# stevenmiller888/mlx-audio

Measured on AMD Instinct MI355X. Metric: audio-sec/sec (xRT), Kokoro-82M batch=32 fixed 128-phoneme utterances per GPU, higher is better.
Workload: dtype bf16; 1 GPU; Kokoro-82M bf16, batch=32/GPU fixed 128-phoneme utterances (T=130, F=650, 390000 samples = 16.25 s each), utterance-sharded over 1 GPU(s); global_batch=32, parallelism=utterance-shard x1, 2 batches in flight per GPU

## Files before the change

include/kokoro_hip.h:

```cpp
#ifndef KOKORO_HIP_H
#define KOKORO_HIP_H

#include <stddef.h>
#include <stdint.h>

#ifdef __cplusplus
extern "C" {
#endif

#define KK_ABI_VERSION 2
#define KK_ABI_MINOR 3

enum { KK_DTYPE_F32 = 0, KK_DTYPE_BF16 = 1, KK_DTYPE_I32 = 2, KK_DTYPE_F16 = 3 };
enum { KK_NOISE_ZERO = 0, KK_NOISE_INJECTED = 1, KK_NOISE_PHILOX = 2 };

typedef struct kk_model kk_model;
typedef struct kk_context kk_context;

typedef struct kk_config {
  int32_t n_token, hidden_dim, style_dim, n_layer, max_dur, text_encoder_kernel_size;
  int32_t plbert_hidden, plbert_heads, plbert_intermediate, plbert_max_pos, plbert_layers, plbert_embedding;
  int32_t decoder_hidden;
  int32_t upsample_initial_channel;
  int32_t n_upsamples;
// ... 23 lines not shown
int kk_forward_text(kk_context* cx, void* stream, int B, int Tmax, const int32_t* ids, const int32_t* lens, const float* ref_s,
                    const float* speed, void* workspace, size_t workspace_bytes, int32_t* pred_dur_out);

int kk_forward_audio(kk_context* cx, void* stream, int B, int Tmax, const int32_t* lens, const float* ref_s, const int32_t* dur, int Fmax,
                     int noise_mode, const float* sine_noise, uint64_t seed, void* workspace, size_t workspace_bytes, float* wav_out,
                     int32_t* nframes_out);

int kk_forward(kk_context* cx, void* stream, int B, int Tmax, const int32_t* ids, const int32_t* lens, const float* ref_s, const float* speed,
               const int32_t* forced_dur, int Fmax, int noise_mode, const float* sine_noise, uint64_t seed, void* workspace,
               size_t workspace_bytes, float* wav_out, int32_t* pred_dur_out, int32_t* nframes_out);

int kk_set_graph_mode(kk_context* cx, int on);

int kk_set_quantization(kk_model* m, int group_size, int bits);
int kk_quantized_layers(const kk_model* m);

const char* kk_last_error(void);
int kk_abi_version(void);
int kk_abi_minor(void);


int kk_op_conv1d(void* stream, int B, const void* x, int ldx, int Lin_rows, const int32_t* lin, const float* w_packed, int ldw,
                 const float* bias, int Cin, int Cout, int Kw, int transposed, int stride, int pad, int dil, int in_shift, float in_slope,
                 int act, float act_slope, const void* res, int ldr, float scale, int accumulate, void* out, int ldo, int Lout_rows,
                 const int32_t* lout, int in_dtype, int out_dtype);
int kk_op_conv1d_bf16(void* stream, int B, const void* x, int ldx, int Lin_rows, const int32_t* lin, const void* w_bf16, int CinP, int CoutP,
                      const float* bias, int Cout, int Kw, int transposed, int stride, int pad, int dil, int in_shift, float in_slope,
                      int act, float act_slope, const void* res, int ldr, float scale, int accumulate, void* out, int ldo, int Lout_rows,
                      const int32_t* lout, int out_dtype);
int kk_op_conv1d_bf16_fused(void* stream, int B, const void* x, int ldx, int L_rows, const int32_t* len, const void* w_bf16, int CinP,
                            int CoutP, const float* bias, int Cin, int Cout, int Kw, int pad, int dil, const float* nrm_a,
                            const float* nrm_b, int nrm_stride, int nrm_act, float nrm_slope, const float* nrm_alpha, const void* res,
                            int ldr, float scale, void* out, int ldo, float* stat_part, int* stat_ntiles_out);
int kk_op_adain(void* stream, int B, const void* x, int ldx, int L_rows, const int32_t* len, int C, const float* gamma_beta, int gbs,
                int act, float slope, const float* alpha, int pool, const float* pool_w, const float* pool_b, void* out, int ldo, int Cpad,
                int Lout_rows, float* scratch, size_t scratch_floats, int dtype, int fast);
int kk_op_layernorm(void* stream, int B, const void* x, int ldx, const void* res, int ldr, int L_rows, const int32_t* len, int C,
                    const float* w, const float* b, const float* gamma_beta, int gbs, float eps, int act, float slope, void* out, int ldo,
                    int dtype);
int kk_op_lstm(void* stream, int B, const float* xproj, const float* whT, int H, int L_rows, const int32_t* len, void* out, int ldo,
               int dtype);
int kk_op_linear_rows(void* stream, int B, const void* x_bf16, long long xbs, int ldx, int rows, const int32_t* len, const void* w_bf16, int N, int K,
                      const float* bias, int act, void* pack_scratch, void* out_bf16, long long obs, int ldo);
int kk_op_lstm_bf16(void* stream, int B, const float* xproj, const void* wh_bf16, int L_rows, const int32_t* len, void* out, int ldo,
                    int dtype);
int kk_op_attention(void* stream, int B, const void* qkv, int ld, int T_rows, const int32_t* len, int heads, void* out, int ldo, int dtype);
int kk_op_source_stft(void* stream, int B, const float* f0, int L2_rows, const int32_t* len2, const float* lin_w9, float lin_b,
                      int noise_mode, const float* noise, uint64_t seed, float* phase_scratch, float* har_source, void* har, int ldhar,
                      int dtype);
int kk_op_istft_head(void* stream, int B, const void* x, int ldx, int Tf_rows, const int32_t* len_frames, float* wav, int dtype, int fast);
int kk_op_pack_head_w(void* stream, const void* w_bf16, void* w_frag);
int kk_op_conv_post_istft(void* stream, int B, const void* x, int ldx, int Tf_rows, const int32_t* len_frames, const void* w_frag,
                          const float* bias, float in_slope, float* wav, void* cp_out, int cp_ld);

int kk_mxfp8_bytes(int rows, int K, size_t* q_bytes, size_t* s_bytes);
int kk_mxfp8_pack_weight(const float* w_host, int N, int K, int group, uint8_t* q_host, uint8_t* s_host);
int kk_op_linear_mxfp8(void* stream, const void* x_bf16, int ldx, int M, int rows_per_item, const int32_t* len, int K, const void* wq,
                       const void* ws, int N, const float* bias, int act, void* aq, void* as, void* out_bf16, int ldo);

int kk_debug_info(kk_context* cx, const char* name, int64_t* rows, int64_t* channels);
int kk_debug_fetch(kk_context* cx, void* stream, const char* name, float* dst);
int kk_debug_override(kk_context* cx, const char* name, const float* src);
void kk_debug_clear(kk_context* cx);
int kk_op_pack_w_frag(void* stream, const void* w_bf16, void* w_frag, int Kw, int CoutP, int CinP);
void kk_debug_set_op_wfrag(const void* w_frag);
void kk_debug_set_op_variant(int v);
// ... 125 lines not shown
```

mlx-audio_amd/_lib.py:

```python
from __future__ import annotations

import ctypes as C
import os

_HERE = os.path.dirname(os.path.abspath(__file__))
LIB_PATH = os.path.join(_HERE, "libkokoro_hip.so")

KK_F32, KK_BF16, KK_I32, KK_F16 = 0, 1, 2, 3
CSM_WEIGHTS = {0: "f32", 1: "bf16", 2: "q8", 3: "q4"}
CSM_WEIGHTS_MIXED, CSM_WEIGHTS_DEQUANTIZED = 0x100, 0x200
NOISE_ZERO, NOISE_INJECTED, NOISE_PHILOX = 0, 1, 2
ACT_NONE, ACT_LRELU, ACT_GELU, ACT_SNAKE = 0, 1, 2, 3


class KKConfig(C.Structure):
    _fields_ = [
        ("n_token", C.c_int32), ("hidden_dim", C.c_int32), ("style_dim", C.c_int32), ("n_layer", C.c_int32),
        ("max_dur", C.c_int32), ("text_encoder_kernel_size", C.c_int32),
        ("plbert_hidden", C.c_int32), ("plbert_heads", C.c_int32), ("plbert_intermediate", C.c_int32),
        ("plbert_max_pos", C.c_int32), ("plbert_layers", C.c_int32), ("plbert_embedding", C.c_int32),
        ("decoder_hidden", C.c_int32), ("upsample_initial_channel", C.c_int32), ("n_upsamples", C.c_int32),
        ("upsample_rates", C.c_int32 * 4), ("upsample_kernel_sizes", C.c_int32 * 4),
        ("n_resblock_kernels", C.c_int32), ("resblock_kernel_sizes", C.c_int32 * 4),
        ("resblock_dilations", (C.c_int32 * 3) * 4),
# ... 17 lines not shown


class KKCsmConfig(C.Structure):
    _fields_ = [("text_vocab_size", C.c_int32), ("audio_vocab_size", C.c_int32), ("audio_num_codebooks", C.c_int32), ("max_seq_len", C.c_int32),
                ("backbone", KKLlamaArgs), ("decoder", KKLlamaArgs)]


class KKCsmSampler(C.Structure):
    _fields_ = [("temperature", C.c_float), ("top_k", C.c_int32), ("top_p", C.c_float), ("min_p", C.c_float), ("min_tokens_to_keep", C.c_int32),
                ("seed", C.c_uint64), ("use_device_rng", C.c_int32)]


_vp, _i, _f, _sz, _u64 = C.c_void_p, C.c_int, C.c_float, C.c_size_t, C.c_uint64
SIGNATURES = {
    "kk_create": (_i, [C.POINTER(KKConfig), C.POINTER(_vp)]),
    "kk_destroy": (None, [_vp]),
    "kk_load_tensor": (_i, [_vp, C.c_char_p, _i, C.POINTER(C.c_int64), _i, _vp]),
    "kk_finalize": (_i, [_vp, _vp]),
    "kk_workspace_bytes": (_sz, [_vp, _i, _i, _i]),
    "kk_context_create": (_i, [_vp, C.POINTER(_vp)]),
    "kk_context_destroy": (None, [_vp]),
    "kk_context_model": (_vp, [_vp]),
    "kk_context_workspace_bytes": (_sz, [_vp, _i, _i, _i]),
    "kk_forward_text": (_i, [_vp, _vp, _i, _i, _vp, _vp, _vp, _vp, _vp, _sz, _vp]),
    "kk_forward_audio": (_i, [_vp, _vp, _i, _i, _vp, _vp, _vp, _i, _i, _vp, _u64, _vp, _sz, _vp, _vp]),
    "kk_forward": (_i, [_vp, _vp, _i, _i, _vp, _vp, _vp, _vp, _vp, _i, _i, _vp, _u64, _vp, _sz, _vp, _vp, _vp]),
    "kk_last_error": (C.c_char_p, []),
    "kk_abi_version": (_i, []),
    "kk_abi_minor": (_i, []),
    "kk_op_conv1d": (_i, [_vp, _i, _vp, _i, _i, _vp, _vp, _i, _vp, _i, _i, _i, _i, _i, _i, _i, _i, _f, _i, _f, _vp, _i, _f, _i, _vp, _i, _i, _vp, _i, _i]),
    "kk_op_conv1d_bf16": (_i, [_vp, _i, _vp, _i, _i, _vp, _vp, _i, _i, _vp, _i, _i, _i, _i, _i, _i, _i, _f, _i, _f, _vp, _i, _f, _i, _vp, _i, _i, _vp, _i]),
    "kk_op_conv1d_bf16_fused": (_i, [_vp, _i, _vp, _i, _i, _vp, _vp, _i, _i, _vp, _i, _i, _i, _i, _i, _vp, _vp, _i, _i, _f, _vp, _vp, _i, _f,
                                     _vp, _i, _vp, C.POINTER(C.c_int)]),
    "kk_op_adain": (_i, [_vp, _i, _vp, _i, _i, _vp, _i, _vp, _i, _i, _f, _vp, _i, _vp, _vp, _vp, _i, _i, _i, _vp, _sz, _i, _i]),
    "kk_op_layernorm": (_i, [_vp, _i, _vp, _i, _vp, _i, _i, _vp, _i, _vp, _vp, _vp, _i, _f, _i, _f, _vp, _i, _i]),
    "kk_op_lstm": (_i, [_vp, _i, _vp, _vp, _i, _i, _vp, _vp, _i, _i]),
    "kk_op_lstm_bf16": (_i, [_vp, _i, _vp, _vp, _i, _vp, _vp, _i, _i]),
    "kk_op_linear_rows": (_i, [_vp, _i, _vp, C.c_longlong, _i, _i, _vp, _vp, _i, _i, _vp, _i, _vp, _vp, C.c_longlong, _i]),
    "kk_op_attention": (_i, [_vp, _i, _vp, _i, _i, _vp, _i, _vp, _i, _i]),
    "kk_op_source_stft": (_i, [_vp, _i, _vp, _i, _vp, _vp, _f, _i, _vp, _u64, _vp, _vp, _vp, _i, _i]),
    "kk_op_istft_head": (_i, [_vp, _i, _vp, _i, _i, _vp, _vp, _i, _i]),
    "kk_op_pack_head_w": (_i, [_vp, _vp, _vp]),
    "kk_op_conv_post_istft": (_i, [_vp, _i, _vp, _i, _i, _vp, _vp, _vp, _f, _vp, _vp, _i]),
    "kk_debug_info": (_i, [_vp, C.c_char_p, C.POINTER(C.c_int64), C.POINTER(C.c_int64)]),
    "kk_debug_fetch": (_i, [_vp, _vp, C.c_char_p, _vp]),
    "kk_debug_override": (_i, [_vp, C.c_char_p, _vp]),
    "kk_debug_clear": (None, [_vp]),
    "kk_debug_force_generic": (None, [_vp, _i]),
    "kk_op_pack_w_frag": (_i, [_vp, _vp, _vp, _i, _i, _i]),
    "kk_csm_create": (_i, [C.POINTER(KKCsmConfig), C.POINTER(_vp)]),
    "kk_csm_destroy": (None, [_vp]),
    "kk_csm_load_tensor": (_i, [_vp, C.c_char_p, C.POINTER(C.c_int64), _i, _vp]),
    "kk_csm_set_weight_dtype": (_i, [_vp, _i]),
    "kk_csm_load_quantized": (_i, [_vp, C.c_char_p, C.POINTER(C.c_int64), _vp, _vp, _vp, _i, _i]),
    "kk_csm_weight_format": (_i, [_vp]),
    "kk_csm_weight_fallback_reason": (C.c_char_p, [_vp]),
    "kk_csm_weight_bytes": (_i, [_vp, C.POINTER(_sz), C.POINTER(_sz)]),
    "kk_csm_finalize": (_i, [_vp, _vp]),
    "kk_csm_share": (_i, [_vp, C.POINTER(_vp)]),
    "kk_csm_setup_caches": (_i, [_vp, _i]),
    "kk_csm_reset_caches": (_i, [_vp]),
    "kk_csm_position": (_i, [_vp]),
    "kk_csm_set_padding": (_i, [_vp, _i, _vp]),
    "kk_csm_workspace_bytes": (_sz, [_vp, _i, _i]),
    "kk_csm_generate_frame": (_i, [_vp, _vp, _i, _i, _vp, _vp, _f, _i, _vp, _vp, _sz, _vp]),
    "kk_csm_generate_frame_ex": (_i, [_vp, _vp, _i, _i, _vp, _vp, C.POINTER(KKCsmSampler), _vp, _vp, _vp, _sz, _vp]),
# ... 96 lines not shown
```

mlx-audio_amd/csrc/kk_conv_mfma5.hip:

```cpp
#include <stdlib.h>

#include "kk_common.h"
#include "kk_kernels.h"
#include "kk_conv_mfma_shared.h"

#ifdef KK_MFMA_TRACE
__device__ unsigned long long kk_mfma5_trace_acc[256][8];
#define TR5_NOW() (__builtin_readcyclecounter())
#define TR5_ADD(slot, v) \
  do { if ((threadIdx.x & 255) == 0) atomicAdd(&kk_mfma5_trace_acc[blockIdx.x & 255][slot], (unsigned long long)(v)); } while (0)
extern "C" int kk_debug_mfma5_trace(unsigned long long* out8, int reset) {
  static unsigned long long h[256][8];
  if (out8) {
    if (hipMemcpyFromSymbol(h, HIP_SYMBOL(kk_mfma5_trace_acc), sizeof(h)) != hipSuccess) return -1;
    for (int k = 0; k < 8; ++k) out8[k] = 0;
    for (int r = 0; r < 256; ++r)
      for (int k = 0; k < 8; ++k) out8[k] += h[r][k];
  }
  if (reset) {
    for (int r = 0; r < 256; ++r)
      for (int k = 0; k < 8; ++k) h[r][k] = 0;
    if (hipMemcpyToSymbol(HIP_SYMBOL(kk_mfma5_trace_acc), h, sizeof(h)) != hipSuccess) return -1;
  }
  return 0;
// ... 261 lines not shown
      unsigned wq[4] = {xreg[i].x & msk & cm[0], xreg[i].y & msk & cm[1], xreg[i].z & msk & cm[2], xreg[i].w & msk & cm[3]};
      if (NRM != 0) {
      } else if (a.in_act == KK_ACT_ELU) {
#pragma unroll
        for (int k = 0; k < 4; ++k) {
          float lo = __uint_as_float(wq[k] << 16), hi = __uint_as_float(wq[k] & 0xFFFF0000u);
          lo = lo > 0.f ? lo : __expf(lo) - 1.0f;
          hi = hi > 0.f ? hi : __expf(hi) - 1.0f;
          const bf16x2 pk = {(bf16_t)lo, (bf16_t)hi};
          wq[k] = __builtin_bit_cast(unsigned, pk);
        }
      } else if (a.in_slope != 1.0f) {
#pragma unroll
        for (int k = 0; k < 4; ++k) {
          float lo = __uint_as_float(wq[k] << 16), hi = __uint_as_float(wq[k] & 0xFFFF0000u);
          lo = lo > 0.f ? lo : lo * a.in_slope;
          hi = hi > 0.f ? hi : hi * a.in_slope;
          const bf16x2 pk = {(bf16_t)lo, (bf16_t)hi};
          wq[k] = __builtin_bit_cast(unsigned, pk);
        }
      }
      xreg[i] = make_uint4(wq[0], wq[1], wq[2], wq[3]);
    }
  };
  auto store_x = [&](const uint4 (&xreg)[XREG]) __attribute__((always_inline)) {
#pragma unroll
    for (int i = 0; i < XREG; ++i) {
      const int id = i * 256 + stid;
      const int r = id >> 3, c8 = (id & 7) * 8;
      if (r < xrows) *(uint4*)(Xs + r * XLD + c8) = xreg[i];
    }
  };

  v2f st_s[4], st_q[4];
  uint4* dump = g_dump5 + (((int)blockIdx.x & 255) << 8) + stid;
  uint4 rres[TPP], rold[ACC ? TPP : 1];
  auto epi_prefetch = [&](const Item& t, int tbase) __attribute__((always_inline)) {
    const bf16_t* ob = (const bf16_t*)a.out + (long long)t.b * a.obs;
    const bf16_t* rb = a.res ? (const bf16_t*)a.res + (long long)t.b * a.rbs : nullptr;
    const int n = t.n0 + (stid & 15) * 8;
    const int nc = n < a.Cout ? n : 0;
    const int lo_hi = a.Lo_rows - 1;
#pragma unroll
    for (int i = 0; i < TPP; ++i) {
      const int q = t.q0 + (tbase + i) * 16 + (stid >> 4);
      const int opc = q < 0 ? 0 : (q > lo_hi ? lo_hi : q);
      if (rb) rres[i] = *(const uint4*)(rb + (long long)opc * a.ldr + nc);
      else rres[i] = make_uint4(0u, 0u, 0u, 0u);
      if (ACC) rold[i] = *(const uint4*)(ob + (long long)opc * a.ldo + nc);
    }
    asm volatile("" ::: "memory");
  };
  auto epi_compute = [&](const Item& t, int tbase) __attribute__((always_inline)) {
    bf16_t* ob = (bf16_t*)a.out + (long long)t.b * a.obs;
    const int n = t.n0 + (stid & 15) * 8;
    const int lo_hi = a.Lo_rows - 1;
    v2f bias2[4];
#pragma unroll
    for (int k = 0; k < 4; ++k) bias2[k] = v2f{s_bias[n + 2 * k], s_bias[n + 2 * k + 1]};
    const v2f scale2 = {a.scale, a.scale}, act_slope2 = {a.act_slope, a.act_slope};
    const bool tile_full = t.live && t.q0 + BM <= t.Lout && t.q0 + BM <= a.Q && t.q0 + BM <= a.Lo_rows && t.n0 + BN <= a.Cout;
    const float* crow = Cs + (tbase * 16 + (stid >> 4)) * CLD + (stid & 15) * 8;
    float4 cn0 = *(const float4*)crow, cn1 = *(const float4*)(crow + 4);
#pragma unroll
    for (int i = 0; i < TPP; ++i) {
      const int row = (tbase + i) * 16 + (stid >> 4);
      const int q = t.q0 + row;
// ... 37 lines not shown
        const unsigned w4[4] = {rres[i].x, rres[i].y, rres[i].z, rres[i].w};
#pragma unroll
        for (int k = 0; k < 4; ++k) v[k] += v2f{__uint_as_float(w4[k] << 16), __uint_as_float(w4[k] & 0xFFFF0000u)};
      }
      if (a.scale != 1.0f) {
#pragma unroll
        for (int k = 0; k < 4; ++k) v[k] *= scale2;
      }
      if (ACC) {
        const unsigned w4[4] = {rold[i].x, rold[i].y, rold[i].z, rold[i].w};
#pragma unroll
        for (int k = 0; k < 4; ++k) v[k] += v2f{__uint_as_float(w4[k] << 16), __uint_as_float(w4[k] & 0xFFFF0000u)};
      }
      if (a.post_slope != 0.f && a.post_slope != 1.0f) {
#pragma unroll
        for (int k = 0; k < 4; ++k) {
          const float mx = v[k].x * a.post_slope, my = v[k].y * a.post_slope;
          v[k].x = v[k].x > mx ? v[k].x : mx;
          v[k].y = v[k].y > my ? v[k].y : my;
        }
      }
      if (!tile_full && !(lv && wr_ok)) {
#pragma unroll
        for (int k = 0; k < 4; ++k) v[k] = v2f{0.f, 0.f};
      }
      unsigned w4[4];
#pragma unroll
      for (int k = 0; k < 4; ++k) {
        const bf16x2 pk = {(bf16_t)v[k].x, (bf16_t)v[k].y};
        w4[k] = __builtin_bit_cast(unsigned, pk);
      }
      uint4* dst = wr_ok ? (uint4*)(ob + (long long)opc * a.ldo + n) : dump;
      *dst = make_uint4(w4[0], w4[1], w4[2], w4[3]);
      if (a.stat_part) {
#pragma unroll
        for (int k = 0; k < 4; ++k) {
          st_s[k] += v[k];
          st_q[k] = fma2(v[k], v[k], st_q[k]);
        }
      }
      asm volatile("" ::: "memory");
    }
  };
  auto stats_reset = [&]() __attribute__((always_inline)) {
#pragma unroll
    for (int k = 0; k < 4; ++k) st_s[k] = st_q[k] = v2f{0.f, 0.f};
  };
  auto stats_to_lds = [&]() __attribute__((always_inline)) {
    float ss[8], sq[8];
#pragma unroll
    for (int k = 0; k < 4; ++k) {
      ss[2 * k] = st_s[k].x; ss[2 * k + 1] = st_s[k].y;
      sq[2 * k] = st_q[k].x; sq[2 * k + 1] = st_q[k].y;
    }
#pragma unroll
    for (int k = 0; k < 8; ++k) {
      ss[k] += __shfl_xor(ss[k], 16);
      ss[k] += __shfl_xor(ss[k], 32);
      sq[k] += __shfl_xor(sq[k], 16);
      sq[k] += __shfl_xor(sq[k], 32);
    }
    if (lane < 16) {
#pragma unroll
      for (int k = 0; k < 8; ++k) {
        red[(swave * 2 + 0) * 128 + lane * 8 + k] = ss[k];
        red[(swave * 2 + 1) * 128 + lane * 8 + k] = sq[k];
      }
    }
  };
  auto stats_to_global = [&](const Item& t) __attribute__((always_inline)) {
    const int which = stid >> 7, col = stid & 127;
    if (t.n0 + col < a.Cout) {
      const float v = red[(0 * 2 + which) * 128 + col] + red[(1 * 2 + which) * 128 + col] + red[(2 * 2 + which) * 128 + col] +
                      red[(3 * 2 + which) * 128 + col];
      const int tile = t.q0 / BM;
      a.stat_part[(((long long)t.b * a.stat_ntiles + tile) * 2 + which) * a.Cout + t.n0 + col] = v;
    }
  };

  auto slab_inside = [&](const Item& t, int chunk) __attribute__((always_inline)) -> bool {
    const int r0 = t.q0 + off0, r1 = t.q0 + off0 + xrows - 1;
    return r0 >= 0 && (a.in_shift ? (r1 >> a.in_shift) : r1) < t.Lin && chunk * CK + CK <= cin_real;
  };
  Item cur = decode(v);
  if (cur.live) {
    load_x(cur, 0, xr0, xk0);
    load_params(cur, 0);
    transform_x(0, xr0, xk0, slab_inside(cur, 0));
    store_x(xr0);
    load_x(cur, 1, xr1, xk1);
  }
  KK_BAR5();
  constexpr int NACT = NTASK / TPP;
  const int act0 = nchunk - NACT;
  Item prev = cur, nxt = cur;
  bool have_prev = false, has_next_item = false;
  auto period = [&](int c, uint4 (&XT)[XREG], unsigned& xkT, uint4 (&XL)[XREG], unsigned& xkL) __attribute__((always_inline)) {
    const bool tail = c == nchunk - 1, tail2 = c + 2 >= nchunk;
    const bool stage1 = tail ? (has_next_item && nxt.live) : cur.live;
    const bool stage2 = tail2 ? (has_next_item && nxt.live) : cur.live;
// ... 3 lines not shown
    const unsigned long long t0 = TR5_NOW();
    load_params(s1, c1);
    load_x(s2, c2, XL, xkL);
    if (!stage2) xkL = 0;
    const unsigned long long t1 = TR5_NOW();
    if (have_prev && c >= act0) {
      epi_compute(prev, (c - act0) * TPP);
      if (tail && a.stat_part) stats_to_lds();
    }
    const unsigned long long t2 = TR5_NOW();
    if (stage1) transform_x(c1, XT, xkT, slab_inside(s1, c1));
    {
      const int tb = tail ? 0 : (c + 1 >= act0 ? (c + 1 - act0) * TPP : 0);
      epi_prefetch(tail ? cur : prev, tb);
    }
    const unsigned long long t3 = TR5_NOW();
    KK_BAR5();
    const unsigned long long t4 = TR5_NOW();
    if (stage1) store_x(XT);
    if (have_prev && tail && a.stat_part) stats_to_global(prev);
    KK_BAR5();
    TR5_ADD(4, t4 - t3);
    TR5_ADD(5, TR5_NOW() - t4);
    TR5_ADD(6, t2 - t1);
    TR5_ADD(7, (t1 - t0) + (t3 - t2));
    (void)t0; (void)t1; (void)t2; (void)t3; (void)t4;
  };
  const unsigned long long trs0 = TR5_NOW();
  (void)trs0;
  for (int j = 0; j < ntile; ++j) {
    cur = decode(v + j * G);
    has_next_item = j + 1 < ntile;
    nxt = has_next_item ? decode(v + (j + 1) * G) : cur;
    if (have_prev) stats_reset();
    for (int c = 0; c < nchunk; c += 2) {
      period(c, xr1, xk1, xr0, xk0);
      period(c + 1, xr0, xk0, xr1, xk1);
    }
    prev = cur;
    have_prev = true;
  }
  TR5_ADD(3, TR5_NOW() - trs0);
  stats_reset();
#pragma unroll
  for (int g = 0; g < NACT; ++g) {
    epi_compute(prev, g * TPP);
    if (g + 1 < NACT) epi_prefetch(prev, (g + 1) * TPP);
  }
  if (a.stat_part) {
    stats_to_lds();
    KK_BAR5();
    stats_to_global(prev);
  }
}

template <int NRM, int TPP, bool ACC>
int launch5(const KKMfmaArgs& a, int B, hipStream_t st) {
  static KKDevOnce attr_once;
  static int ncu_dev[64];
  int dev = 0;
  (void)hipGetDevice(&dev);
  if (attr_once.first()) {
    (void)hipFuncSetAttribute((const void*)conv_mfma5_kernel<NRM, TPP, ACC>, hipFuncAttributeMaxDynamicSharedMemorySize, LDS5_BYTES);
    int n = 0;
    if (hipDeviceGetAttribute(&n, hipDeviceAttributeMultiprocessorCount, dev) != hipSuccess || n <= 0) n = 256;
    ncu_dev[dev & 63] = n;
    attr_once.done();
  }
  const int ncu = ncu_dev[dev & 63];
  const int total = B * kk_cdiv(a.Q, BM) * (a.CoutP / BN);
  const int grid = total < ncu ? total : ncu;
  hipLaunchKernelGGL((conv_mfma5_kernel<NRM, TPP, ACC>), dim3(grid), dim3(512), LDS5_BYTES, st, a, B);
  KK_CHECK_LAUNCH();
  return 0;
}
template <int NRM>
// ... 26 lines not shown
```

mlx-audio_amd/csrc/kk_conv_mfma_epilogue.h:

```cpp
  TO* ob = (TO*)a.out + (long long)b * a.obs;
  const TO* rb = a.res ? (const TO*)a.res + (long long)b * a.rbs : nullptr;
  const int n = n0 + (tid & 15) * 8;
  const int nc = n < a.Cout ? n : 0;
  const int lo_hi = a.Lo_rows - 1;
  constexpr int VEC = sizeof(TO) == 2 ? 1 : 2;
  const bool tile_full = tile_live && !a.flat_T && (a.mode == KK_CONV ? q0 + BM - 1 : phase + a.stride * (q0 + BM - 1)) < Lout;
  v2f bias2[4];
#pragma unroll
  for (int k = 0; k < 4; ++k)
    bias2[k] = a.bias ? v2f{a.bias[n0 + (tid & 15) * 8 + 2 * k], a.bias[n0 + (tid & 15) * 8 + 2 * k + 1]} : v2f{0.f, 0.f};
  const v2f scale2 = {a.scale, a.scale}, act_slope2 = {a.act_slope, a.act_slope};
  v2f st_s[4], st_q[4];
#pragma unroll
  for (int k = 0; k < 4; ++k) st_s[k] = st_q[k] = v2f{0.f, 0.f};

  constexpr int RPP = G::RPP, NPASS = BM / RPP, TASKS = RPP * 16 / 256, TG = TASKS / 2;
  constexpr bool PRE = sizeof(TO) == 2;
  uint4 rpre[PRE ? NPASS * 2 * TG : 1];
  if (PRE && rb) {
#pragma unroll
    for (int j = 0; j < NPASS * 2 * TG; ++j) {
      const int q = q0 + (j / (2 * TG)) * RPP + (((j % (2 * TG)) * 256 + tid) >> 4);
      const int op = a.mode == KK_CONV ? q : phase + a.stride * q;
      const int opc = op < 0 ? 0 : (op > lo_hi ? lo_hi : op);
      rpre[j] = *(const uint4*)(rb + (long long)opc * a.ldr + nc);
    }
    asm volatile("" ::: "memory");
  }
#pragma unroll
  for (int pass = 0; pass < NPASS; ++pass) {
    if (tile_live) {
      if (pass > 0) __syncthreads();
      if (wr == pass) {
        if constexpr (ACC16) {
#pragma unroll
          for (int mi = 0; mi < WM / 16; ++mi)
#pragma unroll
            for (int ni = 0; ni < 4; ++ni) {
              const int col = wc * 64 + ni * 16 + (lane & 15);
              const int rbase = mi * 16 + 4 * (lane >> 4);
#pragma unroll
              for (int r = 0; r < 4; ++r) Cs[(rbase + r) * CLD + col] = acc[mi][ni][r];
            }
        } else {
#pragma unroll
          for (int mi = 0; mi < WM / 32; ++mi)
#pragma unroll
// ... 85 lines not shown
            U32x8 t;
            t.u[0] = rres[i][0];
            t.u[1] = rres[i][VEC - 1];
#pragma unroll
            for (int k = 0; k < 4; ++k) v[k] += v2f{t.f[2 * k], t.f[2 * k + 1]};
          }
        }
        if (a.scale != 1.0f) {
#pragma unroll
          for (int k = 0; k < 4; ++k) v[k] *= scale2;
        }
        if (a.accumulate) {
          if (sizeof(TO) == 2) {
            const unsigned w4[4] = {rold[i][0].x, rold[i][0].y, rold[i][0].z, rold[i][0].w};
#pragma unroll
            for (int k = 0; k < 4; ++k) v[k] += v2f{__uint_as_float(w4[k] << 16), __uint_as_float(w4[k] & 0xFFFF0000u)};
          } else {
            U32x8 t;
            t.u[0] = rold[i][0];
            t.u[1] = rold[i][VEC - 1];
#pragma unroll
            for (int k = 0; k < 4; ++k) v[k] += v2f{t.f[2 * k], t.f[2 * k + 1]};
          }
        }
        if (a.post_slope != 0.f && a.post_slope != 1.0f) {
#pragma unroll
          for (int k = 0; k < 4; ++k) {
            const float mx = v[k].x * a.post_slope, my = v[k].y * a.post_slope;
            v[k].x = v[k].x > mx ? v[k].x : mx;
            v[k].y = v[k].y > my ? v[k].y : my;
          }
        }
        if (sizeof(TO) == 2) {
          if (!tile_full && !live[i]) {
#pragma unroll
            for (int k = 0; k < 4; ++k) v[k] = v2f{0.f, 0.f};
          }
          unsigned w4[4];
#pragma unroll
          for (int k = 0; k < 4; ++k) {
            const bf16x2 pk = {(bf16_t)v[k].x, (bf16_t)v[k].y};
            w4[k] = __builtin_bit_cast(unsigned, pk);
          }
          if (wr_ok[i]) {
            *(uint4*)(ob + (long long)opv[i] * a.ldo + n) = make_uint4(w4[0], w4[1], w4[2], w4[3]);
            if (a.stat_part) {
#pragma unroll
              for (int k = 0; k < 4; ++k) {
                st_s[k] += v[k];
                st_q[k] = fma2(v[k], v[k], st_q[k]);
              }
            }
          }
        } else {
          if (!live[i]) {
#pragma unroll
            for (int k = 0; k < 4; ++k) v[k] = v2f{0.f, 0.f};
          }
          if (wr_ok[i]) {
            float* dst = (float*)(ob + (long long)opv[i] * a.ldo + n);
            *(float4*)dst = make_float4(v[0].x, v[0].y, v[1].x, v[1].y);
            *(float4*)(dst + 4) = make_float4(v[2].x, v[2].y, v[3].x, v[3].y);
          }
        }
      }
    }
    if (pass == 0) TR_ADD(7, TR_NOW() - tr0);
  }
  TR_ADD(4, TR_NOW() - tr0);
  TR_ADD(5, 1);
  if (a.stat_part) {
    __syncthreads();
    float* red = (float*)smem;
    float ss[8], sq[8];
#pragma unroll
    for (int k = 0; k < 4; ++k) {
      ss[2 * k] = st_s[k].x; ss[2 * k + 1] = st_s[k].y;
      sq[2 * k] = st_q[k].x; sq[2 * k + 1] = st_q[k].y;
    }
#pragma unroll
    for (int k = 0; k < 8; ++k) {
      ss[k] += __shfl_xor(ss[k], 16);
      ss[k] += __shfl_xor(ss[k], 32);
      sq[k] += __shfl_xor(sq[k], 16);
      sq[k] += __shfl_xor(sq[k], 32);
    }
    if (lane < 16) {
#pragma unroll
      for (int k = 0; k < 8; ++k) {
        red[(wave * 2 + 0) * 128 + lane * 8 + k] = ss[k];
        red[(wave * 2 + 1) * 128 + lane * 8 + k] = sq[k];
      }
    }
    __syncthreads();
    const int which = tid >> 7, col = tid & 127;
    if (n0 + col < a.Cout) {
      const float v = red[(0 * 2 + which) * 128 + col] + red[(1 * 2 + which) * 128 + col] + red[(2 * 2 + which) * 128 + col] +
                      red[(3 * 2 + which) * 128 + col];
      const int tile = bx * nphase + phase;
      a.stat_part[(((long long)b * a.stat_ntiles + tile) * 2 + which) * a.Cout + n0 + col] = v;
    }
  }
```

mlx-audio_amd/csrc/kk_conv_mfma_shared.h:

```cpp
#pragma once
#include <hip/hip_runtime.h>

namespace {
struct v2f {
  float x, y;
};
__device__ __forceinline__ v2f operator*(v2f a, v2f b) { return v2f{a.x * b.x, a.y * b.y}; }
__device__ __forceinline__ v2f& operator+=(v2f& a, v2f b) { a.x += b.x; a.y += b.y; return a; }
__device__ __forceinline__ v2f& operator*=(v2f& a, v2f b) { a.x *= b.x; a.y *= b.y; return a; }
__device__ __forceinline__ v2f fma2(v2f a, v2f b, v2f c) { return v2f{__builtin_fmaf(a.x, b.x, c.x), __builtin_fmaf(a.y, b.y, c.y)}; }
__device__ __forceinline__ float gelu_exact(float v) { return 0.5f * v * (1.0f + erff(v * 0.70710678118654752440f)); }

typedef float kk_f32x4 __attribute__((ext_vector_type(4)));
typedef __bf16 kk_bf16x8 __attribute__((ext_vector_type(8)));

#define KK_MFMA_KSTEP(KS, B0, B1, B2, B3)                                                                                                  \
  {                                                                                                                                          \
    const kk_bf16x8 b0 = __builtin_bit_cast(kk_bf16x8, B0), b1 = __builtin_bit_cast(kk_bf16x8, B1);                                          \
    const kk_bf16x8 b2 = __builtin_bit_cast(kk_bf16x8, B2), b3 = __builtin_bit_cast(kk_bf16x8, B3);                                          \
    _Pragma("unroll") for (int mi = 0; mi < MI16; ++mi) {                                                                                    \
      const kk_bf16x8 av = *(const kk_bf16x8*)(xa + mi * 16 * XLD + (KS) * 32);                                                              \
      acc[mi][0] = __builtin_amdgcn_mfma_f32_16x16x32_bf16(av, b0, acc[mi][0], 0, 0, 0);                                                     \
      acc[mi][1] = __builtin_amdgcn_mfma_f32_16x16x32_bf16(av, b1, acc[mi][1], 0, 0, 0);                                                     \
      acc[mi][2] = __builtin_amdgcn_mfma_f32_16x16x32_bf16(av, b2, acc[mi][2], 0, 0, 0);                                                     \
      acc[mi][3] = __builtin_amdgcn_mfma_f32_16x16x32_bf16(av, b3, acc[mi][3], 0, 0, 0);                                                     \
    }                                                                                                                                        \
    B0 = fn[((KS) * 4 + 0) * 64];                                                                                                            \
    B1 = fn[((KS) * 4 + 1) * 64];                                                                                                            \
    B2 = fn[((KS) * 4 + 2) * 64];                                                                                                            \
    B3 = fn[((KS) * 4 + 3) * 64];                                                                                                            \
  }
#define KK_MFMA_ITER(Q00, Q01, Q02, Q03, Q10, Q11, Q12, Q13)                                                                               \
  KK_MFMA_KSTEP(0, Q00, Q01, Q02, Q03)                                                                                                     \
  KK_MFMA_KSTEP(1, Q10, Q11, Q12, Q13)                                                                                                     \
  __builtin_amdgcn_sched_group_barrier(0x100, 2, 0);                                                                                         \
  _Pragma("unroll") for (int ks = 0; ks < 2; ++ks) {                                                                                         \
    _Pragma("unroll") for (int j = 0; j < MI16; ++j) {                                                                                       \
      __builtin_amdgcn_sched_group_barrier(0x008, 4, 0);                                                                                     \
      if (ks * MI16 + j + 2 < 2 * MI16) __builtin_amdgcn_sched_group_barrier(0x100, 1, 0);                                                   \
    }                                                                                                                                        \
    __builtin_amdgcn_sched_group_barrier(0x020, 4, 0);                                                                                       \
  }
}
```

mlx-audio_amd/csrc/kk_model.hip:

```cpp
#include <math.h>
#include <stdio.h>
#include <string.h>

#include <algorithm>
#include <functional>
#include <map>
#include <string>
#include <vector>

#include "../../include/kokoro_hip.h"
#include "kk_common.h"
#include "kk_kernels.h"
#include "kk_host.h"

static thread_local std::string g_err;
static const void* g_op_wfrag = nullptr;
static int g_op_variant = 4;

int kk_fail(const char* msg) {
  g_err = msg ? msg : "unknown error";
  return -1;
}
extern "C" const char* kk_last_error(void) { return g_err.c_str(); }
extern "C" int kk_abi_version(void) { return KK_ABI_VERSION; }
// ... 1516 lines not shown
    return rc;
  };
  hipGraphExec_t ex = nullptr;
  KK_TRY(cx->graphs.run(key, st, work, &ex, "kk_forward"));
  if (!ex) return 0;
  KK_TRY(kk_launch_set_u64(cx->seed_dev, seed, st));
  if (hipGraphLaunch(ex, st) != hipSuccess) return kk_fail("kk_forward: hipGraphLaunch failed");
  return 0;
}

extern "C" int kk_set_graph_mode(kk_context* cx, int on) {
  if (!cx) return kk_fail("kk_set_graph_mode: null context");
  cx->graph_mode = on != 0;
  return 0;
}

extern "C" int kk_op_conv1d(void* stream, int B, const void* x, int ldx, int Lin_rows, const int32_t* lin, const float* w_packed, int ldw,
                            const float* bias, int Cin, int Cout, int Kw, int transposed, int stride, int pad, int dil, int in_shift,
                            float in_slope, int act, float act_slope, const void* res, int ldr, float scale, int accumulate, void* out,
                            int ldo, int Lout_rows, const int32_t* lout, int in_dtype, int out_dtype) {
  KKConvArgs a;
  memset(&a, 0, sizeof a);
  a.x = x; a.xbs = (long long)Lin_rows * ldx; a.ldx = ldx; a.w = w_packed; a.ldw = ldw; a.bias = bias;
  a.out = out; a.obs = (long long)Lout_rows * ldo; a.ldo = ldo;
  a.res = res; a.rbs = (long long)Lout_rows * ldr; a.ldr = ldr;
  a.Cin = Cin; a.Cout = Cout; a.Kw = Kw; a.mode = transposed ? KK_CONVT : KK_CONV; a.stride = stride; a.pad = pad; a.dil = dil;
  a.in_shift = in_shift; a.Q = transposed ? kk_cdiv(Lout_rows, stride) : Lout_rows; a.Lo_rows = Lout_rows;
  a.lin = KKLen{lin, lin ? 1 : 0, lin ? 0 : Lin_rows};
  a.lout = KKLen{lout, lout ? 1 : 0, lout ? 0 : Lout_rows};
  a.in_slope = in_slope; a.scale = scale; a.accumulate = accumulate; a.act = act; a.act_slope = act_slope;
  return kk_launch_conv_generic(a, B, in_dtype, out_dtype, (hipStream_t)stream);
}

extern "C" int kk_op_conv1d_bf16(void* stream, int B, const void* x, int ldx, int Lin_rows, const int32_t* lin, const void* w_bf16, int CinP,
                                 int CoutP, const float* bias, int Cout, int Kw, int transposed, int stride, int pad, int dil, int in_shift,
                                 float in_slope, int act, float act_slope, const void* res, int ldr, float scale, int accumulate, void* out,
                                 int ldo, int Lout_rows, const int32_t* lout, int out_dtype) {
  KKMfmaArgs g;
  memset(&g, 0, sizeof g);
  g.x = (const bf16_t*)x; g.xbs = (long long)Lin_rows * ldx; g.ldx = ldx; g.w = (const bf16_t*)w_bf16; g.CinP = CinP; g.CoutP = CoutP; g.bias = bias;
  g.out = out; g.obs = (long long)Lout_rows * ldo; g.ldo = ldo; g.res = res; g.rbs = (long long)Lout_rows * ldr; g.ldr = ldr;
  g.Cout = Cout; g.Kw = Kw; g.mode = transposed ? KK_CONVT : KK_CONV; g.stride = stride; g.pad = pad; g.dil = dil; g.in_shift = in_shift;
  g.Q = transposed ? kk_cdiv(Lout_rows, stride) : Lout_rows; g.Lo_rows = Lout_rows;
  g.lin = KKLen{lin, lin ? 1 : 0, lin ? 0 : Lin_rows};
  g.lout = KKLen{lout, lout ? 1 : 0, lout ? 0 : Lout_rows};
  g.in_slope = in_slope; g.scale = scale; g.accumulate = accumulate; g.act = act; g.act_slope = act_slope;
  if (!kk_mfma_eligible(CinP, Cout, Kw, g.mode, stride, dil)) return kk_fail("kk_op_conv1d_bf16: shape not eligible for the MFMA kernel");
  if (g_op_wfrag && out_dtype == KK_BF16) {
    g.wf = (const bf16_t*)g_op_wfrag;
    if (g_op_variant == 5 && kk_mfma5_eligible(g, out_dtype)) return kk_launch_conv_mfma5(g, B, out_dtype, (hipStream_t)stream);
    return kk_launch_conv_mfma4(g, B, out_dtype, (hipStream_t)stream);
  }
  return kk_launch_conv_mfma(g, B, out_dtype, (hipStream_t)stream);
}

extern "C" int kk_op_conv1d_bf16_fused(void* stream, int B, const void* x, int ldx, int L_rows, const int32_t* len, const void* w_bf16, int CinP,
                                       int CoutP, const float* bias, int Cin, int Cout, int Kw, int pad, int dil, const float* nrm_a,
                                       const float* nrm_b, int nrm_stride, int nrm_act, float nrm_slope, const float* nrm_alpha,
                                       const void* res, int ldr, float scale, void* out, int ldo, float* stat_part, int* stat_ntiles_out) {
  KKMfmaArgs g;
  memset(&g, 0, sizeof g);
  g.x = (const bf16_t*)x; g.xbs = (long long)L_rows * ldx; g.ldx = ldx; g.w = (const bf16_t*)w_bf16; g.CinP = CinP; g.Cin = Cin; g.CoutP = CoutP; g.bias = bias;
  g.out = out; g.obs = (long long)L_rows * ldo; g.ldo = ldo; g.res = res; g.rbs = (long long)L_rows * ldr; g.ldr = ldr;
  g.Cout = Cout; g.Kw = Kw; g.mode = KK_CONV; g.stride = 1; g.pad = pad; g.dil = dil; g.Q = L_rows; g.Lo_rows = L_rows;
  g.lin = KKLen{len, len ? 1 : 0, len ? 0 : L_rows};
  g.lout = g.lin;
  g.in_slope = 1.f; g.scale = scale;
  g.nrm_a = nrm_a; g.nrm_b = nrm_b; g.nrm_stride = nrm_stride; g.nrm_act = nrm_act; g.nrm_slope = nrm_slope; g.nrm_alpha = nrm_alpha; g.nrm_C = Cin;
  g.stat_part = stat_part;
  g.stat_ntiles = kk_cdiv(L_rows, KK_MFMA_TILE_ROWS);
  if (stat_ntiles_out) *stat_ntiles_out = g.stat_ntiles;
  if (!kk_mfma_eligible(CinP, Cout, Kw, KK_CONV, 1, dil)) return kk_fail("kk_op_conv1d_bf16_fused: shape not eligible for the MFMA kernel");
  if (g_op_wfrag) {
    g.wf = (const bf16_t*)g_op_wfrag;
    if (g_op_variant == 5 && kk_mfma5_eligible(g, KK_BF16)) return kk_launch_conv_mfma5(g, B, KK_BF16, (hipStream_t)stream);
    return kk_launch_conv_mfma4(g, B, KK_BF16, (hipStream_t)stream);
  }
  return kk_launch_conv_mfma(g, B, KK_BF16, (hipStream_t)stream);
}

extern "C" int kk_op_adain(void* stream, int B, const void* x, int ldx, int L_rows, const int32_t* len, int C, const float* gamma_beta,
                           int gbs, int act, float slope, const float* alpha, int pool, const float* pool_w, const float* pool_b, void* out,
                           int ldo, int Cpad, int Lout_rows, float* scratch, size_t scratch_floats, int dtype, int fast) {
  const size_t np = kk_stats_partial_floats(B, C, L_rows, 512);
  if (scratch_floats < np + 2 * (size_t)B * C) return kk_fail("kk_op_adain: scratch too small");
  KKStatsArgs s;
// ... 212 lines not shown
```

Baseline: 15010 audio-sec/sec.

## Compute conv epilogue channel statistics with MFMA over LDS-staged bf16 tiles

Replaces the per-thread running sum and sum-of-squares accumulation (plus shuffle reductions) in the conv epilogues with a scheme that stages the packed bf16 outputs in LDS. It then reads them back with transposed LDS loads and reduces them using MFMA: a ones-vector product gives the column sums and a self-product diagonal gives the sums of squares. The aim is to take the statistics arithmetic and cross-lane shuffles off the vector ALUs. In exchange it adds LDS traffic, an extra barrier per pass, and statistics computed from bf16-rounded values rather than fp32. It also adds a standalone conv+stats op entry point and tightens the full-tile condition.

```diff
diff --git a/include/kokoro_hip.h b/include/kokoro_hip.h
--- a/include/kokoro_hip.h
+++ b/include/kokoro_hip.h
@@ -79,6 +79,9 @@
                             int CoutP, const float* bias, int Cin, int Cout, int Kw, int pad, int dil, const float* nrm_a,
                             const float* nrm_b, int nrm_stride, int nrm_act, float nrm_slope, const float* nrm_alpha, const void* res,
                             int ldr, float scale, void* out, int ldo, float* stat_part, int* stat_ntiles_out);
+int kk_op_conv1d_bf16_stats(void* stream, int B, const void* x, int ldx, int Lin_rows, const int32_t* lin, const void* w_bf16, int CinP,
+                            int CoutP, const float* bias, int Cout, int Kw, int transposed, int stride, int pad, int dil, const void* res,
+                            int ldr, void* out, int ldo, int Lout_rows, const int32_t* lout, float* stat_part, int* stat_ntiles_out);
 int kk_op_adain(void* stream, int B, const void* x, int ldx, int L_rows, const int32_t* len, int C, const float* gamma_beta, int gbs,
                 int act, float slope, const float* alpha, int pool, const float* pool_w, const float* pool_b, void* out, int ldo, int Cpad,
                 int Lout_rows, float* scratch, size_t scratch_floats, int dtype, int fast);
diff --git a/mlx-audio_amd/_lib.py b/mlx-audio_amd/_lib.py
--- a/mlx-audio_amd/_lib.py
+++ b/mlx-audio_amd/_lib.py
@@ -73,6 +73,7 @@
     "kk_op_conv1d_bf16": (_i, [_vp, _i, _vp, _i, _i, _vp, _vp, _i, _i, _vp, _i, _i, _i, _i, _i, _i, _i, _f, _i, _f, _vp, _i, _f, _i, _vp, _i, _i, _vp, _i]),
     "kk_op_conv1d_bf16_fused": (_i, [_vp, _i, _vp, _i, _i, _vp, _vp, _i, _i, _vp, _i, _i, _i, _i, _i, _vp, _vp, _i, _i, _f, _vp, _vp, _i, _f,
                                      _vp, _i, _vp, C.POINTER(C.c_int)]),
+    "kk_op_conv1d_bf16_stats": (_i, [_vp, _i, _vp, _i, _i, _vp, _vp, _i, _i, _vp, _i, _i, _i, _i, _i, _i, _vp, _i, _vp, _i, _i, _vp, _vp, C.POINTER(C.c_int)]),
     "kk_op_adain": (_i, [_vp, _i, _vp, _i, _i, _vp, _i, _vp, _i, _i, _f, _vp, _i, _vp, _vp, _vp, _i, _i, _i, _vp, _sz, _i, _i]),
     "kk_op_layernorm": (_i, [_vp, _i, _vp, _i, _vp, _i, _i, _vp, _i, _vp, _vp, _vp, _i, _f, _i, _f, _vp, _i, _i]),
     "kk_op_lstm": (_i, [_vp, _i, _vp, _vp, _i, _i, _vp, _vp, _i, _i]),
diff --git a/mlx-audio_amd/csrc/kk_conv_mfma5.hip b/mlx-audio_amd/csrc/kk_conv_mfma5.hip
--- a/mlx-audio_amd/csrc/kk_conv_mfma5.hip
+++ b/mlx-audio_amd/csrc/kk_conv_mfma5.hip
@@ -317,7 +317,6 @@
     }
   };
 
-  v2f st_s[4], st_q[4];
   uint4* dump = g_dump5 + (((int)blockIdx.x & 255) << 8) + stid;
   uint4 rres[TPP], rold[ACC ? TPP : 1];
   auto epi_prefetch = [&](const Item& t, int tbase) __attribute__((always_inline)) {
@@ -421,40 +420,24 @@
       }
       uint4* dst = wr_ok ? (uint4*)(ob + (long long)opc * a.ldo + n) : dump;
       *dst = make_uint4(w4[0], w4[1], w4[2], w4[3]);
-      if (a.stat_part) {
-#pragma unroll
-        for (int k = 0; k < 4; ++k) {
-          st_s[k] += v[k];
-          st_q[k] = fma2(v[k], v[k], st_q[k]);
-        }
-      }
+      if (a.stat_part) *(uint4*)((unsigned char*)Cs + kk_stat_word_off(row, stid & 15, CLD * 4)) = make_uint4(w4[0], w4[1], w4[2], w4[3]);
       asm volatile("" ::: "memory");
     }
   };
-  auto stats_reset = [&]() __attribute__((always_inline)) {
-#pragma unroll
-    for (int k = 0; k < 4; ++k) st_s[k] = st_q[k] = v2f{0.f, 0.f};
-  };
   auto stats_to_lds = [&]() __attribute__((always_inline)) {
-    float ss[8], sq[8];
-#pragma unroll
-    for (int k = 0; k < 4; ++k) {
-      ss[2 * k] = st_s[k].x; ss[2 * k + 1] = st_s[k].y;
-      sq[2 * k] = st_q[k].x; sq[2 * k + 1] = st_q[k].y;
-    }
-#pragma unroll
-    for (int k = 0; k < 8; ++k) {
-      ss[k] += __shfl_xor(ss[k], 16);
-      ss[k] += __shfl_xor(ss[k], 32);
-      sq[k] += __shfl_xor(sq[k], 16);
-      sq[k] += __shfl_xor(sq[k], 32);
-    }
-    if (lane < 16) {
-#pragma unroll
-      for (int k = 0; k < 8; ++k) {
-        red[(swave * 2 + 0) * 128 + lane * 8 + k] = ss[k];
-        red[(swave * 2 + 1) * 128 + lane * 8 + k] = sq[k];
-      }
+    const unsigned char* tb = (const unsigned char*)Cs + kk_stat_lane_off((lane >> 4) * 16 + swave * 4 + ((lane >> 2) & 3), lane, CLD * 4);
+    const __bf16 z = (__bf16)0.0f;
+#pragma unroll
+    for (int cb = 0; cb < BN / 16; ++cb) {
+      const kk_bf16x4 r0 = kk_lds_read_tr16(tb + cb * 64);
+      const kk_bf16x4 r1 = kk_lds_read_tr16(tb + 64 * CLD * 4 + cb * 64);
+      const kk_bf16x4 r2 = kk_lds_read_tr16(tb + 128 * CLD * 4 + cb * 64);
+      kk_f32x4 ds = {0.f, 0.f, 0.f, 0.f}, dq = {0.f, 0.f, 0.f, 0.f};
+      kk_stat_mfma(kk_stat_frag(r0, r1), ds, dq);
+      kk_stat_mfma(kk_stat_frag(r2, kk_bf16x4{z, z, z, z}), ds, dq);
+      const float q = kk_stat_diag(dq, lane);
+      if (lane < 16) red[(swave * 2 + 0) * 128 + cb * 16 + lane] = ds[0];
+      if (kk_stat_diag_lane(lane)) red[(swave * 2 + 1) * 128 + cb * 16 + (lane & 15)] = q;
     }
   };
   auto stats_to_global = [&](const Item& t) __attribute__((always_inline)) {
@@ -524,7 +507,6 @@
     cur = decode(v + j * G);
     has_next_item = j + 1 < ntile;
     nxt = has_next_item ? decode(v + (j + 1) * G) : cur;
-    if (have_prev) stats_reset();
     for (int c = 0; c < nchunk; c += 2) {
       period(c, xr1, xk1, xr0, xk0);
       period(c + 1, xr0, xk0, xr1, xk1);
@@ -533,7 +515,6 @@
     have_prev = true;
   }
   TR5_ADD(3, TR5_NOW() - trs0);
-  stats_reset();
 #pragma unroll
   for (int g = 0; g < NACT; ++g) {
     epi_compute(prev, g * TPP);
diff --git a/mlx-audio_amd/csrc/kk_conv_mfma_epilogue.h b/mlx-audio_amd/csrc/kk_conv_mfma_epilogue.h
--- a/mlx-audio_amd/csrc/kk_conv_mfma_epilogue.h
+++ b/mlx-audio_amd/csrc/kk_conv_mfma_epilogue.h
@@ -4,15 +4,18 @@
   const int nc = n < a.Cout ? n : 0;
   const int lo_hi = a.Lo_rows - 1;
   constexpr int VEC = sizeof(TO) == 2 ? 1 : 2;
-  const bool tile_full = tile_live && !a.flat_T && (a.mode == KK_CONV ? q0 + BM - 1 : phase + a.stride * (q0 + BM - 1)) < Lout;
+  const int op_last = a.mode == KK_CONV ? q0 + BM - 1 : phase + a.stride * (q0 + BM - 1);
+  const bool tile_full = tile_live && !a.flat_T && op_last < Lout && q0 + BM <= a.Q && op_last < a.Lo_rows && n0 + BN <= a.Cout;
   v2f bias2[4];
 #pragma unroll
   for (int k = 0; k < 4; ++k)
     bias2[k] = a.bias ? v2f{a.bias[n0 + (tid & 15) * 8 + 2 * k], a.bias[n0 + (tid & 15) * 8 + 2 * k + 1]} : v2f{0.f, 0.f};
   const v2f scale2 = {a.scale, a.scale}, act_slope2 = {a.act_slope, a.act_slope};
-  v2f st_s[4], st_q[4];
-#pragma unroll
-  for (int k = 0; k < 4; ++k) st_s[k] = st_q[k] = v2f{0.f, 0.f};
+  constexpr bool STAT = sizeof(TO) == 2;
+  const bool stat_mm = STAT && a.stat_part && tile_live;
+  kk_f32x4 sd_s[2], sd_q[2];
+#pragma unroll
+  for (int j = 0; j < 2; ++j) sd_s[j] = sd_q[j] = kk_f32x4{0.f, 0.f, 0.f, 0.f};
 
   constexpr int RPP = G::RPP, NPASS = BM / RPP, TASKS = RPP * 16 / 256, TG = TASKS / 2;
   constexpr bool PRE = sizeof(TO) == 2;
@@ -164,7 +167,7 @@
           }
         }
         if (sizeof(TO) == 2) {
-          if (!tile_full && !live[i]) {
+          if (!tile_full && !(live[i] && wr_ok[i])) {
 #pragma unroll
             for (int k = 0; k < 4; ++k) v[k] = v2f{0.f, 0.f};
           }
@@ -174,16 +177,8 @@
             const bf16x2 pk = {(bf16_t)v[k].x, (bf16_t)v[k].y};
             w4[k] = __builtin_bit_cast(unsigned, pk);
           }
-          if (wr_ok[i]) {
-            *(uint4*)(ob + (long long)opv[i] * a.ldo + n) = make_uint4(w4[0], w4[1], w4[2], w4[3]);
-            if (a.stat_part) {
-#pragma unroll
-              for (int k = 0; k < 4; ++k) {
-                st_s[k] += v[k];
-                st_q[k] = fma2(v[k], v[k], st_q[k]);
-              }
-            }
-          }
+          if (wr_ok[i]) *(uint4*)(ob + (long long)opv[i] * a.ldo + n) = make_uint4(w4[0], w4[1], w4[2], w4[3]);
+          if (stat_mm) *(uint4*)((unsigned char*)Cs + kk_stat_word_off(row, tid & 15, CLD * 4)) = make_uint4(w4[0], w4[1], w4[2], w4[3]);
         } else {
           if (!live[i]) {
 #pragma unroll
@@ -196,40 +191,32 @@
           }
         }
       }
+    }
+    if (stat_mm) {
+      __syncthreads();
+      const unsigned char* tb = (const unsigned char*)Cs + kk_stat_lane_off((lane >> 4) * 4 + ((lane >> 2) & 3), lane, CLD * 4) + wave * 128;
+#pragma unroll
+      for (int kb = 0; kb < RPP / 32; ++kb)
+#pragma unroll
+        for (int j = 0; j < 2; ++j) {
+          const kk_bf16x4 lo = kk_lds_read_tr16(tb + (kb * 32) * CLD * 4 + j * 64);
+          const kk_bf16x4 hi = kk_lds_read_tr16(tb + (kb * 32 + 16) * CLD * 4 + j * 64);
+          kk_stat_mfma(kk_stat_frag(lo, hi), sd_s[j], sd_q[j]);
+        }
     }
     if (pass == 0) TR_ADD(7, TR_NOW() - tr0);
   }
   TR_ADD(4, TR_NOW() - tr0);
   TR_ADD(5, 1);
   if (a.stat_part) {
-    __syncthreads();
-    float* red = (float*)smem;
-    float ss[8], sq[8];
-#pragma unroll
-    for (int k = 0; k < 4; ++k) {
-      ss[2 * k] = st_s[k].x; ss[2 * k + 1] = st_s[k].y;
-      sq[2 * k] = st_q[k].x; sq[2 * k + 1] = st_q[k].y;
-    }
-#pragma unroll
-    for (int k = 0; k < 8; ++k) {
-      ss[k] += __shfl_xor(ss[k], 16);
-      ss[k] += __shfl_xor(ss[k], 32);
-      sq[k] += __shfl_xor(sq[k], 16);
-      sq[k] += __shfl_xor(sq[k], 32);
-    }
-    if (lane < 16) {
-#pragma unroll
-      for (int k = 0; k < 8; ++k) {
-        red[(wave * 2 + 0) * 128 + lane * 8 + k] = ss[k];
-        red[(wave * 2 + 1) * 128 + lane * 8 + k] = sq[k];
-      }
-    }
-    __syncthreads();
-    const int which = tid >> 7, col = tid & 127;
-    if (n0 + col < a.Cout) {
-      const float v = red[(0 * 2 + which) * 128 + col] + red[(1 * 2 + which) * 128 + col] + red[(2 * 2 + which) * 128 + col] +
-                      red[(3 * 2 + which) * 128 + col];
-      const int tile = bx * nphase + phase;
-      a.stat_part[(((long long)b * a.stat_ntiles + tile) * 2 + which) * a.Cout + n0 + col] = v;
+    static_assert(RPP % 32 == 0, "the statistics walk the pass in 32-row blocks");
+    const int tile = bx * nphase + phase;
+    float* sp = a.stat_part + ((long long)b * a.stat_ntiles + tile) * 2 * a.Cout;
+#pragma unroll
+    for (int j = 0; j < 2; ++j) {
+      const int col = n0 + wave * 32 + j * 16 + (lane & 15);
+      const float dq = kk_stat_diag(sd_q[j], lane);
+      if (lane < 16 && col < a.Cout) sp[col] = sd_s[j][0];
+      if (kk_stat_diag_lane(lane) && col < a.Cout) sp[a.Cout + col] = dq;
     }
   }
diff --git a/mlx-audio_amd/csrc/kk_conv_mfma_shared.h b/mlx-audio_amd/csrc/kk_conv_mfma_shared.h
--- a/mlx-audio_amd/csrc/kk_conv_mfma_shared.h
+++ b/mlx-audio_amd/csrc/kk_conv_mfma_shared.h
@@ -13,6 +13,29 @@
 
 typedef float kk_f32x4 __attribute__((ext_vector_type(4)));
 typedef __bf16 kk_bf16x8 __attribute__((ext_vector_type(8)));
+typedef __bf16 kk_bf16x4 __attribute__((ext_vector_type(4)));
+
+__device__ __forceinline__ int kk_stat_word_off(int row, int chunk, int pitch_bytes) { return row * pitch_bytes + chunk * 32 + (row & 1) * 16; }
+__device__ __forceinline__ int kk_stat_lane_off(int row, int lane, int pitch_bytes) {
+  return kk_stat_word_off(row, (lane & 3) >> 1, pitch_bytes) + (lane & 1) * 8;
+}
+__device__ __forceinline__ kk_bf16x4 kk_lds_read_tr16(const unsigned char* p) {
+  return __builtin_amdgcn_ds_read_tr16_b64_v4bf16((__attribute__((address_space(3))) kk_bf16x4*)p);
+}
+__device__ __forceinline__ kk_bf16x8 kk_stat_frag(kk_bf16x4 lo, kk_bf16x4 hi) {
+  return kk_bf16x8{lo[0], lo[1], lo[2], lo[3], hi[0], hi[1], hi[2], hi[3]};
+}
+__device__ __forceinline__ void kk_stat_mfma(kk_bf16x8 f, kk_f32x4& s, kk_f32x4& sq) {
+  const __bf16 one = (__bf16)1.0f;
+  const kk_bf16x8 ones = {one, one, one, one, one, one, one, one};
+  sq = __builtin_amdgcn_mfma_f32_16x16x32_bf16(f, f, sq, 0, 0, 0);
+  s = __builtin_amdgcn_mfma_f32_16x16x32_bf16(ones, f, s, 0, 0, 0);
+}
+__device__ __forceinline__ bool kk_stat_diag_lane(int lane) { return (lane >> 4) == ((lane & 15) >> 2); }
+__device__ __forceinline__ float kk_stat_diag(kk_f32x4 d, int lane) {
+  const int r = lane & 3;
+  return r == 0 ? d[0] : r == 1 ? d[1] : r == 2 ? d[2] : d[3];
+}
 
 #define KK_MFMA_KSTEP(KS, B0, B1, B2, B3)                                                                                                  \
   {                                                                                                                                          \
diff --git a/mlx-audio_amd/csrc/kk_model.hip b/mlx-audio_amd/csrc/kk_model.hip
--- a/mlx-audio_amd/csrc/kk_model.hip
+++ b/mlx-audio_amd/csrc/kk_model.hip
@@ -1572,10 +1572,10 @@
   return kk_launch_conv_generic(a, B, in_dtype, out_dtype, (hipStream_t)stream);
 }
 
-extern "C" int kk_op_conv1d_bf16(void* stream, int B, const void* x, int ldx, int Lin_rows, const int32_t* lin, const void* w_bf16, int CinP,
-                                 int CoutP, const float* bias, int Cout, int Kw, int transposed, int stride, int pad, int dil, int in_shift,
-                                 float in_slope, int act, float act_slope, const void* res, int ldr, float scale, int accumulate, void* out,
-                                 int ldo, int Lout_rows, const int32_t* lout, int out_dtype) {
+static int op_conv1d_bf16(void* stream, int B, const void* x, int ldx, int Lin_rows, const int32_t* lin, const void* w_bf16, int CinP, int CoutP,
+                          const float* bias, int Cout, int Kw, int transposed, int stride, int pad, int dil, int in_shift, float in_slope, int act,
+                          float act_slope, const void* res, int ldr, float scale, int accumulate, void* out, int ldo, int Lout_rows,
+                          const int32_t* lout, int out_dtype, float* stat_part, int* stat_ntiles_out) {
   KKMfmaArgs g;
   memset(&g, 0, sizeof g);
   g.x = (const bf16_t*)x; g.xbs = (long long)Lin_rows * ldx; g.ldx = ldx; g.w = (const bf16_t*)w_bf16; g.CinP = CinP; g.CoutP = CoutP; g.bias = bias;
@@ -1585,6 +1585,11 @@
   g.lin = KKLen{lin, lin ? 1 : 0, lin ? 0 : Lin_rows};
   g.lout = KKLen{lout, lout ? 1 : 0, lout ? 0 : Lout_rows};
   g.in_slope = in_slope; g.scale = scale; g.accumulate = accumulate; g.act = act; g.act_slope = act_slope;
+  if (stat_part) {
+    g.stat_part = stat_part;
+    g.stat_ntiles = kk_cdiv(g.Q, KK_MFMA_TILE_ROWS) * (transposed ? stride : 1);
+    if (stat_ntiles_out) *stat_ntiles_out = g.stat_ntiles;
+  }
   if (!kk_mfma_eligible(CinP, Cout, Kw, g.mode, stride, dil)) return kk_fail("kk_op_conv1d_bf16: shape not eligible for the MFMA kernel");
   if (g_op_wfrag && out_dtype == KK_BF16) {
     g.wf = (const bf16_t*)g_op_wfrag;
@@ -1592,6 +1597,22 @@
     return kk_launch_conv_mfma4(g, B, out_dtype, (hipStream_t)stream);
   }
   return kk_launch_conv_mfma(g, B, out_dtype, (hipStream_t)stream);
+}
+
+extern "C" int kk_op_conv1d_bf16(void* stream, int B, const void* x, int ldx, int Lin_rows, const int32_t* lin, const void* w_bf16, int CinP,
+                                 int CoutP, const float* bias, int Cout, int Kw, int transposed, int stride, int pad, int dil, int in_shift,
+                                 float in_slope, int act, float act_slope, const void* res, int ldr, float scale, int accumulate, void* out,
+                                 int ldo, int Lout_rows, const int32_t* lout, int out_dtype) {
+  return op_conv1d_bf16(stream, B, x, ldx, Lin_rows, lin, w_bf16, CinP, CoutP, bias, Cout, Kw, transposed, stride, pad, dil, in_shift, in_slope, act,
+                        act_slope, res, ldr, scale, accumulate, out, ldo, Lout_rows, lout, out_dtype, nullptr, nullptr);
+}
+
+extern "C" int kk_op_conv1d_bf16_stats(void* stream, int B, const void* x, int ldx, int Lin_rows, const int32_t* lin, const void* w_bf16, int CinP,
+                                       int CoutP, const float* bias, int Cout, int Kw, int transposed, int stride, int pad, int dil, const void* res,
+                                       int ldr, void* out, int ldo, int Lout_rows, const int32_t* lout, float* stat_part, int* stat_ntiles_out) {
+  if (!stat_part) return kk_fail("kk_op_conv1d_bf16_stats: stat_part missing");
+  return op_conv1d_bf16(stream, B, x, ldx, Lin_rows, lin, w_bf16, CinP, CoutP, bias, Cout, Kw, transposed, stride, pad, dil, 0, 1.f, KK_ACT_NONE, 0.f,
+                        res, ldr, 1.f, 0, out, ldo, Lout_rows, lout, KK_BF16, stat_part, stat_ntiles_out);
 }
 
 extern "C" int kk_op_conv1d_bf16_fused(void* stream, int B, const void* x, int ldx, int L_rows, const int32_t* len, const void* w_bf16, int CinP,
```

Result: slower. 14820 audio-sec/sec (-1.3%).
